# dluvizon/deephar

Measured on NVIDIA H100. Metric: frames/sec (256x256, 16-frame clips, b32), higher is better.
Workload: dtype bf16x3 split (fp32 accumulate, wgmma)

## Files before the change

### deephar_b200/_ffi.py

```python
import ctypes as C
import os

_HERE = os.path.dirname(os.path.abspath(__file__))
LIB_PATH = os.environ.get('DEEPHAR_B200_LIB') or os.path.join(_HERE, 'libdeephar_b200.so')


class DeepharB200Error(RuntimeError):
    pass


class dh_view(C.Structure):
    _fields_ = [('p', C.c_void_p), ('n', C.c_int32), ('h', C.c_int32), ('w', C.c_int32),
                ('c', C.c_int32), ('ld', C.c_int32)]


class dh_conv_desc(C.Structure):
    _fields_ = [('kh', C.c_int32), ('kw', C.c_int32), ('sh', C.c_int32), ('sw', C.c_int32),
                ('pad_same', C.c_int32), ('pre_relu', C.c_int32), ('post_relu', C.c_int32),
                ('n_res', C.c_int32),
                ('pre_scale', C.c_void_p), ('pre_shift', C.c_void_p),
                ('post_scale', C.c_void_p), ('post_shift', C.c_void_p),
                ('res', dh_view * 2),
                ('precision', C.c_int32), ('res_up2x', C.c_int32), ('pool_out', dh_view)]


class dh_frame_src(C.Structure):
    _fields_ = [('data', C.c_uint64), ('h', C.c_int32), ('w', C.c_int32), ('stride', C.c_int32),
                ('x0', C.c_int32), ('y0', C.c_int32), ('cw', C.c_int32), ('ch', C.c_int32), ('hflip', C.c_int32),
                ('kx_off', C.c_int32), ('ky_off', C.c_int32), ('kx_coef_off', C.c_int32), ('ky_coef_off', C.c_int32),
                ('ksx', C.c_int32), ('ksy', C.c_int32)]


class dh_packed_w(C.Structure):
    _fields_ = [('hi', C.c_void_p), ('lo', C.c_void_p), ('cout_pad', C.c_int32), ('k', C.c_int32)]


class dh_conv_plan_info(C.Structure):
    _fields_ = [('path', C.c_int32), ('fallback', C.c_int32), ('workspace_bytes', C.c_int64),
                ('n_mtiles', C.c_int32), ('grid_x', C.c_int32), ('grid_y', C.c_int32), ('bn_cta', C.c_int32),
                ('n_kblocks', C.c_int32), ('stages', C.c_int32), ('cluster', C.c_int32)]


class dh_clip_window(C.Structure):
    _fields_ = [('src', dh_view), ('dst', dh_view), ('ring', C.c_void_p)]


class dh_jpeg_image(C.Structure):
    _fields_ = [('data', C.c_int64), ('coef', C.c_int64 * 3), ('plane', C.c_int64 * 3), ('out', C.c_int64),
                ('h', C.c_int32), ('w', C.c_int32), ('ncomp', C.c_int32), ('hs', C.c_int32), ('vs', C.c_int32),
                ('mcus_x', C.c_int32), ('mcus_y', C.c_int32), ('bw', C.c_int32 * 3), ('bh', C.c_int32 * 3),
                ('qt', C.c_int32 * 3), ('dc', C.c_int32 * 3), ('ac', C.c_int32 * 3), ('nblocks', C.c_int32),
                ('pad', C.c_int32)]


class dh_jpeg_segment(C.Structure):
# ... 111 lines not shown
```

### deephar_b200/csrc/conv_api.cu

```cuda
#include "tc_common.cuh"

namespace {

struct Choice {
    DhConvPath path;
    bool fallback;
    int64_t workspace_bytes;
    tc::PatchPlan patch;
    tc::SepPlan sep;
    tc::TcPlan tcp;
};

int choose_conv(const dh_ctx* ctx, const ConvParams& p, const dh_packed_w* packed, bool separable, int precision,
                Choice* c) {
    const bool packed_hi = packed && packed->hi;
    c->fallback = false;
    c->workspace_bytes = 0;
    if (separable) {
        DH_CHECK_ARG(!p.pool, "dh_sepconv2d_f32: pool_out is not supported by the separable kernels");
        if (packed_hi && dh_plan_sep_tma(ctx, p, packed, precision, &c->sep)) { c->path = DH_PATH_SEP_TMA; return 0; }
    } else {
        if (!p.up1 && !p.pool && dh_conv_smallk_ok(p)) { c->path = DH_PATH_SIMT; return 0; }
        if (ctx->pw_smallk && !p.up1 && dh_pw_smallk_supported(p)) { c->path = DH_PATH_PW_SMALLK; return 0; }
        DH_CHECK_ARG(!p.pool, "dh_conv2d_f32: pool_out is written by the wide pointwise kernel only (1x1, stride 1, "
// ... 47 lines not shown
    q.kh = q.kw = 1; q.sh = q.sw = 1; q.pt = q.pl = 0;
    q.pre_scale = q.pre_shift = nullptr; q.pre_relu = 0;
    q.K = p.Cin;
    dh_launch_conv_simt(q, s);
    DH_LAUNCH_EPILOGUE(ctx, 2);
}

template <class Params>
void tc_info(const dh_ctx* ctx, const tc::Plan<Params>& pl, const tc::TcParams& P, dh_conv_plan_info* info) {
    info->n_mtiles = P.n_mtiles;
    info->grid_x = tc::persistent_gx(ctx, pl.gy, P.n_mtiles);
    info->grid_y = pl.gy;
    info->bn_cta = P.bn_cta;
    info->n_kblocks = P.n_kblocks;
    info->cluster = pl.cluster;
}

int plan_info(const dh_ctx* ctx, const Choice& c, dh_conv_plan_info* info) {
    DH_CHECK_ARG(info, "dh_conv_plan_info: NULL info");
    *info = dh_conv_plan_info{};
    info->path = c.path;
    info->fallback = c.fallback;
    info->workspace_bytes = c.workspace_bytes;
    if (c.path == DH_PATH_TC) {
        tc_info(ctx, c.tcp, c.tcp.k, info);
        info->stages = c.tcp.k.stages;
    }
    if (c.path == DH_PATH_SEP_TMA) tc_info(ctx, c.sep, c.sep.k.t, info);
    if (c.path == DH_PATH_PATCH) tc_info(ctx, c.patch, c.patch.k.t, info);
    return 0;
}

}

extern "C" int dh_conv2d_f32(dh_ctx* ctx, const dh_view* x, const float* w_hwio,
                             const dh_packed_w* packed, const dh_conv_desc* d, const dh_view* out,
                             void* stream) {
    ConvParams p;
    Choice c;
    int rc = plan_conv(ctx, x, nullptr, w_hwio, packed, d, out, false, &p, &c);
    return rc ? rc : launch_choice(ctx, p, c, false, (cudaStream_t)stream);
}

// ... 26 lines not shown
```

### deephar_b200/csrc/conv_sep.cu

```cuda
#include "tc_common.cuh"

namespace tcs {
using namespace tc;
using R = tc::Roles<2, 1>;
constexpr int WARP_EPI0 = R::WARP_EPI0, WARP_TMA = R::WARP_TMA, WARP_PATCH = R::WARP_PATCH, NTHREADS = R::NTHREADS,
              REGS_PROD = R::REGS_PROD, REGS_EPI = R::REGS_EPI, REGS_CTRL = R::REGS_CTRL;

constexpr int NWG = 128;
constexpr int NPW = 1;
constexpr int NA = 4;
constexpr int NB = 3;
constexpr int NP = 3;

template <int KS, int TW, bool SHARE, bool BNPRO, bool LO>
__global__ void __launch_bounds__(NTHREADS, 1)
sep_tma_kernel(const __grid_constant__ SepParams SP, const __grid_constant__ CUtensorMap map_hi,
               const __grid_constant__ CUtensorMap map_lo, const __grid_constant__ CUtensorMap map_x) {
    constexpr int PAD = KS / 2;
    constexpr int PC = TW + 2 * PAD;
    constexpr int NR = 4 + KS - 1;
#ifdef DH_ABLATE
    const int DBG = SP.dbg;
#else
    constexpr int DBG = 0;
#endif
    const TcParams& P = SP.t;
    extern __shared__ __align__(1024) uint8_t smem_raw[];
    if (smem_u32(smem_raw) & 1023u) __trap();
    uint8_t* smem = smem_raw;
    const int tid = threadIdx.x;
    const int warp = tid >> 5, lane = tid & 31;
    constexpr bool want_lo = LO;
    const int b_bytes = P.bn_cta * 64;
    uint8_t* b_ring = smem + NA * 2 * A_BYTES;
    uint8_t* patch0 = b_ring + NB * 2 * b_bytes;
// ... 30 lines not shown
    if (SHARE) cluster_sync_all(); else __syncthreads();

    const int tiles_mine = ((int)P.n_mtiles - (int)blockIdx.x + (int)gridDim.x - 1) / (int)gridDim.x;
    const int total_g = tiles_mine * nkb;
    const int n_own = SHARE ? (total_g - (int)my_rank + 1) / 2 : total_g;

    if (warp < WARP_EPI0) {
        reg_prod<REGS_PROD, R::LAUNCH_REGS>();
        const ConvParams& c = P.c;
        const int w = warp >> 2;
        const int tw = tid & (NWG - 1);
        const int cp = tw & 15;
        const int blk = tw >> 4;
        constexpr int XB = TW / 4;
        const int strip = blk / XB, xb = blk - strip * XB;
        const int fn = (strip * 4) / SP.ry, ry = (strip * 4) - fn * SP.ry;
        const int prr = SP.ry + 2 * PAD;
        const float* pbase0 = reinterpret_cast<const float*>(patch0) +
                             ((size_t)((fn * prr + ry) * PC + xb * 4)) * SBK + cp * 2;
        const int row0 = strip * 4 * TW + xb * 4;
        const float lowb = c.pre_relu ? 0.f : -3.402823466e38f;
        unsigned colmask = 0;
        if (BNPRO) {
#pragma unroll
            for (int q = 0; q < NR; ++q) {
                const int ix = xb * 4 + q - PAD;
                if (ix >= 0 && ix < TW) colmask |= 1u << q;
            }
        }
        float2 wt[KS][KS];
        auto load_taps = [&](int jn) {
            const int gn = SHARE ? 2 * jn + (int)my_rank : jn;
            const int kbn = gn % nkb;
            const float* wp = c.w_dw + kbn * SBK + cp * 2;
#pragma unroll
            for (int a = 0; a < KS; ++a)
#pragma unroll
                for (int b = 0; b < KS; ++b)
                    wt[a][b] = __ldg(reinterpret_cast<const float2*>(wp + (size_t)(a * KS + b) * c.Cin));
        };
        if (w < n_own) load_taps(w);
        for (int j = w; j < n_own; j += NPW) {
            const int pb_i = j % NP;
            const uint32_t pfull = bar_pfull0 + 8 * pb_i, pempty = bar_pempty0 + 8 * pb_i;
            const float* pbase = pbase0 + (size_t)pb_i * (SP.patch_stride / 4);
            const int g = SHARE ? 2 * j + (int)my_rank : j;
            const int ti = g / nkb, kb = g - ti * nkb;
            const int ch = kb * SBK + cp * 2;
            float2 acc[4][4];
#pragma unroll
            for (int o = 0; o < 4; ++o)
#pragma unroll
                for (int q = 0; q < 4; ++q) acc[o][q] = make_float2(0.f, 0.f);
            float2 ps = make_float2(1.f, 1.f), pb = make_float2(0.f, 0.f);
            unsigned rowmask = 0;
            if (BNPRO) {
                ps = __ldg(reinterpret_cast<const float2*>(c.pre_scale + ch));
                pb = __ldg(reinterpret_cast<const float2*>(c.pre_shift + ch));
                const int t = blockIdx.x + ti * gridDim.x;
                const int y0 = SP.fn > 1 ? 0 : ((t * BM) / TW) % c.H;
#pragma unroll
                for (int r = 0; r < NR; ++r) {
                    const int iy = y0 + ry + r - PAD;
                    if (iy >= 0 && iy < c.H) rowmask |= 1u << r;
                }
            }

            if (!(DBG & 2)) mbar_wait_relaxed(pfull, (uint32_t)((j / NP) & 1), (DBG & 2048) ? 32u : 0u);
            auto load_row = [&](int r, float2* in) {
#pragma unroll
                for (int q = 0; q < NR; ++q) {
                    float2 v = *reinterpret_cast<const float2*>(pbase + (r * PC + q) * SBK);
                    if (BNPRO) v = ffma2(v, ps, pb);
                    v = make_float2(fmaxf(v.x, lowb), fmaxf(v.y, lowb));
                    if (BNPRO && !(((rowmask >> r) & 1u) && ((colmask >> q) & 1u))) v = make_float2(0.f, 0.f);
                    in[q] = v;
                }
            };
            if (!(DBG & 1)) {
                float2 inb[2][NR];
                load_row(0, inb[0]);
#pragma unroll
                for (int r = 0; r < NR; ++r) {
                    if (r + 1 < NR) load_row(r + 1, inb[(r + 1) & 1]);
                    const float2* in = inb[r & 1];
#pragma unroll
                    for (int kx = 0; kx < KS; ++kx)
#pragma unroll
                        for (int o = 0; o < 4; ++o) {
                            const int ky = r - o;
                            if (ky >= 0 && ky < KS) {
#pragma unroll
                                for (int q = 0; q < 4; ++q) acc[o][q] = ffma2(wt[ky][kx], in[q + kx], acc[o][q]);
                            }
                        }
                }
            }
            if (j + NPW < n_own) load_taps(j + NPW);
            if (!(DBG & 2)) mbar_arrive(pempty);

            const int s = g % NA;
            const uint32_t it = (uint32_t)(g / NA);
            wait_stage_free(bar_empty0, s, it, (DBG & 2048) ? 32u : 0u);
            uint8_t* a_hi = smem + (size_t)s * (2 * A_BYTES);
            uint8_t* a_lo = a_hi + A_BYTES;
#pragma unroll
            for (int o = 0; o < 4; ++o)
#pragma unroll
                for (int q = 0; q < 4; ++q) {
                    uint32_t hi, lo;
                    split2(acc[o][q].x, acc[o][q].y, hi, lo);
                    const uint32_t off = swz64(row0 + o * TW + q, cp * 2);
                    *reinterpret_cast<uint32_t*>(a_hi + off) = hi;
                    if (want_lo) *reinterpret_cast<uint32_t*>(a_lo + off) = lo;
                }
            fence_proxy_async();
            if (SHARE) {
                asm volatile("bar.sync %0, %1;" ::"r"(1 + w), "r"(NWG) : "memory");
                if (tw == 0) {
                    mbar_arrive(bar_full0 + 8 * s);
                    const uint32_t peer = my_rank ^ 1u;
                    const uint32_t peer_full = mapa_peer(bar_full0 + 8 * s, peer);
                    if (!(DBG & 8)) {
                        bulk_s2peer(mapa_peer(smem_u32(a_hi), peer), smem_u32(a_hi), A_BYTES, peer_full);
                        if (want_lo) bulk_s2peer(mapa_peer(smem_u32(a_lo), peer), smem_u32(a_lo), A_BYTES, peer_full);
                    }
                }
            } else {
                mbar_arrive(bar_full0 + 8 * s);
            }
        }
    } else if (warp < WARP_TMA) {
        reg_inc<REGS_EPI>();
        stage_post<R::NEPI>(P, n0, post, tid - 32 * WARP_EPI0);
        const int wg = (warp - WARP_EPI0) >> 2, wt = tid - 32 * WARP_EPI0 - 128 * wg;
        pp_consumer<SHARE, LO, NA, NB>(P, wg, wt, n0, tiles_mine, make_desc64(smem_u32(smem)), make_desc64(smem_u32(b_ring)),
                                       bar_full0, bar_empty0, bar_fullb0, bar_emptyb0, my_rank, post, DBG);
    } else {
        reg_dec<REGS_CTRL>();
        if (warp == WARP_TMA) {
            if (lane == 0) {
                const uint32_t tx = (DBG & 16) ? 0u : (uint32_t)(want_lo ? 2 : 1) * (uint32_t)b_bytes;
                const uint32_t tx_a = (DBG & 8) ? 0u : (uint32_t)(want_lo ? 2 : 1) * (uint32_t)A_BYTES;
                for (int g = 0; g < total_g; ++g) {
                    const int ti = g / nkb, kb = g - ti * nkb;
                    const int sb = g % NB;
                    const uint32_t itb = (uint32_t)(g / NB);
                    if (itb >= 1) mbar_wait_relaxed(bar_emptyb0 + 8 * sb, (itb - 1) & 1, (DBG & 2048) ? 64u : 0u);
                    const uint32_t full = bar_fullb0 + 8 * sb;
                    mbar_arrive_expect_tx(full, tx);
                    const uint32_t b_hi = smem_u32(b_ring + (size_t)sb * (2 * b_bytes));
// ... 5 lines not shown
                    if (SHARE && (uint32_t)(g & 1) != my_rank) {
                        const int sa = g % NA;
                        wait_stage_free(bar_empty0, sa, (uint32_t)(g / NA));
                        mbar_arrive_expect_tx(bar_full0 + 8 * sa, tx_a);
                    }
                }
            }
        } else if (warp == WARP_PATCH) {
            if (lane == 0 && !(DBG & 2)) {
                const ConvParams& c = P.c;
                auto coords = [&](int j, int& kb, int& nf, int& y0) {
                    const int g = SHARE ? 2 * j + (int)my_rank : j;
                    const int ti = g / nkb;
                    kb = g - ti * nkb;
                    const int t = blockIdx.x + ti * gridDim.x;
                    const int grow = (t * BM) / TW;
                    nf = grow / c.H;
                    y0 = grow - nf * c.H;
                };
                for (int j = 0; j < n_own; ++j) {
                    int kb, nf, y0;
                    coords(j, kb, nf, y0);
                    const int w = j % NP;
                    const int pfd = (DBG & 1024) ? 2 : (DBG & 4096) ? 4 : (DBG & 8192) ? 9 : 0;
                    if (pfd && j + pfd < n_own) {
                        int kb2, nf2, y2;
                        coords(j + pfd, kb2, nf2, y2);
                        tma_prefetch_4d(&map_x, kb2 * SBK, -PAD, y2 - PAD, nf2);
                    }
                    mbar_wait_relaxed(bar_pempty0 + 8 * w, (uint32_t)(((j / NP) & 1) ^ 1), (DBG & 2048) ? 64u : 0u);
                    const uint32_t pf = bar_pfull0 + 8 * w;
// ... 4 lines not shown
        }
    }
    if (SHARE) cluster_sync_all(); else __syncthreads();
}

}

bool dh_plan_sep_tma(const dh_ctx* ctx, const ConvParams& p, const dh_packed_w* packed, int precision, tc::SepPlan* pl) {
    using namespace tc;
    using namespace tcs;
    if (!ctx->sep_tma || !packed->lo || !sep_layer_ok(p, packed)) return false;
    if (!(p.W == 32 || p.W == 16 || p.W == 8)) return false;
    const int tr = BM / p.W;
    if (tr <= p.H ? (p.H % tr) != 0 : (tr % p.H) != 0) return false;
    if ((p.Cin % SBK) != 0 || (p.ldx & 3)) return false;
    SepParams& SP = pl->k;
    TcParams& P = SP.t;
    P.c = p;
    P.c.K = p.Cin;
    P.k_pad = packed->k;
    P.n_kblocks = p.Cin / SBK;
    int gy;
    tile_n(p.Cout, &P.bn_cta, &gy);
    P.precision = (precision == 1) ? 1 : 3;
    P.ks = p.kh;
    P.n_mtiles = (p.M + BM - 1) / BM;
    P.stages = 2;
    const int pad = p.kh / 2;
    SP.ry = tr <= p.H ? tr : p.H;
    SP.fn = tr <= p.H ? 1 : tr / p.H;
    SP.patch_bytes = SBK * 4 * (p.W + 2 * pad) * (SP.ry + 2 * pad) * SP.fn;
    SP.patch_stride = (SP.patch_bytes + 1023) / 1024 * 1024;
#ifdef DH_ABLATE
    SP.dbg = ctx->dbg;
    P.dbg = ctx->dbg;
#else
    SP.dbg = 0;
    P.dbg = 0;
#endif
    pl->smem = (size_t)NA * 2 * A_BYTES + (size_t)NB * 2 * P.bn_cta * 64 + NP * (size_t)SP.patch_stride + 512 +
               POST_SMEM;
    if (pl->smem > SMEM_LIMIT) return false;
    pl->w = packed;
    pl->gy = gy;
    pl->cluster = gy % 2 == 0 && ctx->share_a;
    return true;
}

int dh_launch_sep_tma(const dh_ctx* ctx, const tc::SepPlan& pl, cudaStream_t s) {
    using namespace tc;
    using namespace tcs;
    const TcParams& P = pl.k.t;
    const ConvParams& c = P.c;
    const dh_packed_w* w = pl.w;
    const int pad = P.ks / 2;
    CUtensorMap map_hi, map_lo, map_x;
    if (!make_map_w(&map_hi, w->hi, w->k, w->cout_pad, SBK, P.bn_cta) ||
        !make_map_w(&map_lo, w->lo, w->k, w->cout_pad, SBK, P.bn_cta) ||
        !make_map_x(&map_x, c.x, c.ldx, c.Cin, c.W, c.H, c.N, c.W + 2 * pad, pl.k.ry + 2 * pad, pl.k.fn)) {
        dh_set_error("dh_launch_sep_tma: cuTensorMapEncodeTiled failed");
        return -1;
    }
    return pick<5, 3>(P.ks, [&](auto ks) {
        return pick<32, 16, 8>(c.W, [&](auto tw) {
            return pick<true, false>(pl.cluster, [&](auto share) {
                return pick<true, false>(c.pre_scale != nullptr, [&](auto bnpro) {
                    return pick<true, false>(P.precision == 3, [&](auto lo) {
                        return launch_persistent<sep_tma_kernel<ks(), tw(), share(), bnpro(), lo()>>(
                            "dh_launch_sep_tma", ctx, pl, P.n_mtiles, NTHREADS, s, map_hi, map_lo, map_x);
                    });
                });
            });
        });
    });
}
```

### deephar_b200/csrc/tc_common.cuh

```cuda
#pragma once
#include <cuda.h>
#include <cuda_bf16.h>
#include <type_traits>
#include "common.cuh"
#include "conv_params.cuh"

namespace tc {


constexpr int BM = 128;
constexpr int BK = 64;
constexpr int NPROD = 256;
constexpr int MAX_BN_CTA = 96;
constexpr int ACC_N = MAX_BN_CTA / 2;
constexpr int MH = BM / 64;
template <int Q, int NPW = 2>
struct Roles {
    static constexpr int EPQ = Q;
    static constexpr int NEPI = 128 * Q;
    static constexpr int WARP_EPI0 = 4 * NPW;
    static constexpr int WARP_TMA = WARP_EPI0 + 4 * Q, WARP_PATCH = WARP_TMA + 2;
    static constexpr int NTHREADS = 32 * (WARP_TMA + 4);
    static constexpr int REGS_PROD = Q == 1 ? 168 : (NPW == 1 ? 192 : 88);
    static constexpr int REGS_EPI = Q == 2 && NPW == 2 ? 136 : 144, REGS_CTRL = 32;
    static constexpr int LAUNCH_REGS = NTHREADS <= 512 ? 128 : 96;
    static_assert(128 * NPW * REGS_PROD + NEPI * REGS_EPI + 128 * REGS_CTRL <= NTHREADS * LAUNCH_REGS,
                  "setmaxnreg budget exceeds the CTA's register allocation: the last setmaxnreg.inc would never return");
};
constexpr int A_TILE_BYTES = BM * 128;
constexpr int MAX_STAGES = 4;
// ... 3 lines not shown
    int n_kblocks;
    int bn_cta;
    int stages;
    int precision;
    int ks;
    int k_pad;
    int n_mtiles;
    int dbg;
};

struct SepParams {
    TcParams t;
    int patch_stride;
    int patch_bytes;
    int ry, fn;
    int dbg;
};

struct PatchParams {
    TcParams t;
    int np, patch_stride, patch_bytes;
    int ntaps, ncb;
    int tw;
    int ry, fn;
    int pc, pr;
    int rows_per_frame;
    int kw;
    int pt, pl, sh, sw;
    int vh, vw;
    int mask;
// ... 73 lines not shown
template <> __device__ __forceinline__ void wgmma_bf16<80>(float* d, uint64_t a, uint64_t b, uint32_t acc) {
    asm volatile(
        "{\n .reg .pred p;\n setp.ne.b32 p, %42, 0;\n"
        " wgmma.mma_async.sync.aligned.m64n80k16.f32.bf16.bf16 {%0, %1, %2, %3, %4, %5, %6, %7, %8, %9, %10, %11, %12, %13, %14, %15, %16, %17, %18, %19, %20, %21, %22, %23, %24, %25, %26, %27, %28, %29, %30, %31, %32, %33, %34, %35, %36, %37, %38, %39}, %40, %41, p, 1, 1, 0, 0;\n}"
        : "+f"(d[0]), "+f"(d[1]), "+f"(d[2]), "+f"(d[3]), "+f"(d[4]), "+f"(d[5]), "+f"(d[6]), "+f"(d[7]), "+f"(d[8]), "+f"(d[9]), "+f"(d[10]), "+f"(d[11]), "+f"(d[12]), "+f"(d[13]), "+f"(d[14]), "+f"(d[15]), "+f"(d[16]), "+f"(d[17]), "+f"(d[18]), "+f"(d[19]), "+f"(d[20]), "+f"(d[21]), "+f"(d[22]), "+f"(d[23]), "+f"(d[24]), "+f"(d[25]), "+f"(d[26]), "+f"(d[27]), "+f"(d[28]), "+f"(d[29]), "+f"(d[30]), "+f"(d[31]), "+f"(d[32]), "+f"(d[33]), "+f"(d[34]), "+f"(d[35]), "+f"(d[36]), "+f"(d[37]), "+f"(d[38]), "+f"(d[39])
        : "l"(a), "l"(b), "r"(acc));
}
template <> __device__ __forceinline__ void wgmma_bf16<96>(float* d, uint64_t a, uint64_t b, uint32_t acc) {
    asm volatile(
        "{\n .reg .pred p;\n setp.ne.b32 p, %50, 0;\n"
        " wgmma.mma_async.sync.aligned.m64n96k16.f32.bf16.bf16 {%0, %1, %2, %3, %4, %5, %6, %7, %8, %9, %10, %11, %12, %13, %14, %15, %16, %17, %18, %19, %20, %21, %22, %23, %24, %25, %26, %27, %28, %29, %30, %31, %32, %33, %34, %35, %36, %37, %38, %39, %40, %41, %42, %43, %44, %45, %46, %47}, %48, %49, p, 1, 1, 0, 0;\n}"
        : "+f"(d[0]), "+f"(d[1]), "+f"(d[2]), "+f"(d[3]), "+f"(d[4]), "+f"(d[5]), "+f"(d[6]), "+f"(d[7]), "+f"(d[8]), "+f"(d[9]), "+f"(d[10]), "+f"(d[11]), "+f"(d[12]), "+f"(d[13]), "+f"(d[14]), "+f"(d[15]), "+f"(d[16]), "+f"(d[17]), "+f"(d[18]), "+f"(d[19]), "+f"(d[20]), "+f"(d[21]), "+f"(d[22]), "+f"(d[23]), "+f"(d[24]), "+f"(d[25]), "+f"(d[26]), "+f"(d[27]), "+f"(d[28]), "+f"(d[29]), "+f"(d[30]), "+f"(d[31]), "+f"(d[32]), "+f"(d[33]), "+f"(d[34]), "+f"(d[35]), "+f"(d[36]), "+f"(d[37]), "+f"(d[38]), "+f"(d[39]), "+f"(d[40]), "+f"(d[41]), "+f"(d[42]), "+f"(d[43]), "+f"(d[44]), "+f"(d[45]), "+f"(d[46]), "+f"(d[47])
        : "l"(a), "l"(b), "r"(acc));
}

__device__ __forceinline__ uint64_t make_desc(uint32_t smem_addr) {
    return (uint64_t)((smem_addr >> 4) & 0x3FFF) | (1ull << 16) | ((uint64_t)(1024 >> 4) << 32) | (1ull << 62);
}


__device__ __forceinline__ void split2(float a, float b, uint32_t& hi, uint32_t& lo) {
    __nv_bfloat162 h = __floats2bfloat162_rn(a, b);
    float ra = a - __low2float(h), rb = b - __high2float(h);
    __nv_bfloat162 l = __floats2bfloat162_rn(ra, rb);
    hi = *reinterpret_cast<uint32_t*>(&h);
    lo = *reinterpret_cast<uint32_t*>(&l);
}

__device__ __forceinline__ uint32_t swz(int row, int k) {
    return (uint32_t)(row * 128 + ((((k >> 3) ^ (row & 7)) << 4) | ((k & 7) << 1)));
// ... 21 lines not shown
__device__ __forceinline__ uint32_t swz64(int row, int k) {
    return (uint32_t)(row * 64 + ((((k >> 3) ^ ((row >> 1) & 3)) << 4) | ((k & 7) << 1)));
}

__device__ __forceinline__ float4 lds128(uint32_t a) {
    float4 v;
    asm volatile("ld.shared.v4.f32 {%0, %1, %2, %3}, [%4];" : "=f"(v.x), "=f"(v.y), "=f"(v.z), "=f"(v.w) : "r"(a) : "memory");
    return v;
}

__device__ __forceinline__ void wait_stage_free(uint32_t bar_empty0, int s, uint32_t it, uint32_t ns = 0) {
    if (it >= 1) mbar_wait_relaxed(bar_empty0 + 16 * s + 8 * ((it - 1) & 1), ((it - 1) >> 1) & 1, ns);
}


template <int N>
__device__ __forceinline__ void acc_fence_all(float (&acc)[MH][ACC_N]) {
#pragma unroll
    for (int h = 0; h < MH; ++h)
#pragma unroll
        for (int i = 0; i < N / 2; ++i) acc_fence(acc[h][i]);
}

template <int N, int NK16, bool LO>
__device__ __forceinline__ void wg_issue_kblock(float (&acc)[MH][ACC_N], uint64_t da, uint32_t a_half16, uint32_t alo16,
                                                uint64_t db, uint32_t blo16, bool first) {
    wgmma_fence();
#pragma unroll
    for (int k = 0; k < NK16; ++k) {
        const uint32_t acc0 = (first && k == 0) ? 0u : 1u;
#pragma unroll
        for (int h = 0; h < MH; ++h) {
            const uint64_t a = da + (uint64_t)(h * a_half16 + 2 * k);
            wgmma_bf16<N>(acc[h], a, db + 2 * k, acc0);
            if (LO) {
                wgmma_bf16<N>(acc[h], a + alo16, db + 2 * k, 1u);
                wgmma_bf16<N>(acc[h], a, db + blo16 + 2 * k, 1u);
            }
        }
    }
    wgmma_commit();
}

template <int N, int NK16, bool LO, class Stage, class Release>
__device__ __forceinline__ void wg_tile_n(float (&acc)[MH][ACC_N], int nkb, uint32_t a_half16, uint32_t alo16,
                                          uint32_t blo16, bool mma, Stage& stage, Release& release) {
    for (int kb = 0; kb < nkb; ++kb) {
        uint64_t da, db;
        stage(kb, da, db);
        if (mma) {
            acc_fence_all<N>(acc);
            wg_issue_kblock<N, NK16, LO>(acc, da, a_half16, alo16, db, blo16, kb == 0);
        }
        wgmma_wait<1>();
        acc_fence_all<N>(acc);
        if (kb > 0) release(kb - 1);
    }
    wgmma_wait<0>();
    acc_fence_all<N>(acc);
    release(nkb - 1);
}

template <int NK16, bool LO, class Stage, class Release>
__device__ __forceinline__ void wg_tile(int bn, float (&acc)[MH][ACC_N], int nkb, uint32_t a_half16, uint32_t alo16,
                                        uint32_t blo16, bool mma, Stage&& stage, Release&& release) {
    switch (bn) {
    case 16: wg_tile_n<16, NK16, LO>(acc, nkb, a_half16, alo16, blo16, mma, stage, release); break;
    case 32: wg_tile_n<32, NK16, LO>(acc, nkb, a_half16, alo16, blo16, mma, stage, release); break;
    case 48: wg_tile_n<48, NK16, LO>(acc, nkb, a_half16, alo16, blo16, mma, stage, release); break;
    case 64: wg_tile_n<64, NK16, LO>(acc, nkb, a_half16, alo16, blo16, mma, stage, release); break;
    case 80: wg_tile_n<80, NK16, LO>(acc, nkb, a_half16, alo16, blo16, mma, stage, release); break;
    default: wg_tile_n<96, NK16, LO>(acc, nkb, a_half16, alo16, blo16, mma, stage, release); break;
    }
}

__device__ __forceinline__ void pp_pass(int wg) { asm volatile("bar.arrive %0, 256;" ::"r"(6 + wg) : "memory"); }
__device__ __forceinline__ void pp_wait(int wg) { asm volatile("bar.sync %0, 256;" ::"r"(7 - wg) : "memory"); }

__device__ __forceinline__ void wg_release(uint32_t bar, int wg, int wt, bool remote, uint32_t peer) {
    asm volatile("bar.sync %0, 128;" ::"r"(4 + wg) : "memory");
    if (wt == 0) {
        mbar_arrive(bar);
        if (remote) mbar_arrive_cluster(mapa_peer(bar, peer));
    }
}

__device__ __forceinline__ size_t res1_src(const ConvParams& c, int m) {
    if (!c.up1) return (size_t)m;
    const int hw = c.Ho * c.Wo;
    const int n = m / hw, rem = m - n * hw;
    const int y = rem / c.Wo, x = rem - y * c.Wo;
    return ((size_t)n * (c.Ho >> 1) + (y >> 1)) * (size_t)(c.Wo >> 1) + (size_t)(x >> 1);
}

__device__ __forceinline__ float2 ldg2(const float* p) { return __ldg(reinterpret_cast<const float2*>(p)); }

constexpr int POST_SMEM = 2 * MAX_BN_CTA * 4;
template <int NEPI>
__device__ __forceinline__ void stage_post(const TcParams& P, int n0, float* post, int ct) {
    const ConvParams& c = P.c;
    if (c.post_scale) {
        for (int j = ct; j < P.bn_cta; j += NEPI) {
            const int co = n0 + j;
            post[j] = co < c.Cout ? __ldg(c.post_scale + co) : 0.f;
            post[MAX_BN_CTA + j] = co < c.Cout ? __ldg(c.post_shift + co) : 0.f;
        }
    }
    asm volatile("bar.sync 2, %0;" ::"n"(NEPI) : "memory");
}

__device__ __forceinline__ void prefetch_l2(const float* p) { asm volatile("prefetch.global.L2 [%0];" ::"l"(p)); }
__device__ __forceinline__ void wg_prefetch_res(const TcParams& P, int m0, int n0, int wt) {
    const ConvParams& c = P.c;
#ifdef DH_ABLATE
    if (P.dbg & 32) return;
#endif
    const int m = m0 + wt;
    if (m >= c.M) return;
    const int last = min(P.bn_cta, c.Cout - n0) - 1;
    if (c.res0) {
        const float* r = c.res0 + (size_t)m * c.ldr0 + n0;
        for (int k = 0; k < last; k += 32) prefetch_l2(r + k);
        prefetch_l2(r + last);
    }
    if (c.res1) {
        const float* r = c.res1 + res1_src(c, m) * c.ldr1 + n0;
        for (int k = 0; k < last; k += 32) prefetch_l2(r + k);
        prefetch_l2(r + last);
    }
}

__device__ __forceinline__ void wg_epilogue(const TcParams& P, const float (&acc)[MH][ACC_N], int m0, int n0, int wt,
                                            const float* post) {
    const ConvParams& c = P.c;
#ifdef DH_ABLATE
    if (P.dbg & 32) return;
#endif
    const int rq = 16 * (wt >> 5) + ((wt & 31) >> 2);
    const int c0 = n0 + 2 * (wt & 3);
    const bool v2 = !((c.ldo | c.Cout) & 1) && !(reinterpret_cast<uintptr_t>(c.out) & 7) &&
                    (!c.res0 || (!(c.ldr0 & 1) && !(reinterpret_cast<uintptr_t>(c.res0) & 7))) &&
                    (!c.res1 || (!(c.ldr1 & 1) && !(reinterpret_cast<uintptr_t>(c.res1) & 7)));
    const bool relu = c.post_relu != 0, has_post = c.post_scale != nullptr;
    const int ncol = min(P.bn_cta - 2 * (wt & 3), c.Cout - c0);
    const float* sc = post + (c0 - n0);
    const float* sh = sc + MAX_BN_CTA;
    constexpr int JC = 3;
    static_assert((ACC_N / 4) % JC == 0, "column groups per batch");
#pragma unroll
    for (int h = 0; h < MH; ++h)
#pragma unroll
        for (int hr = 0; hr < 2; ++hr) {
            const int m = m0 + 64 * h + rq + 8 * hr;
            if (m >= c.M) continue;
            float* orow = c.out + (size_t)m * c.ldo + c0;
            const float* r0row = c.res0 ? c.res0 + (size_t)m * c.ldr0 + c0 : nullptr;
            const float* r1row = c.res1 ? c.res1 + res1_src(c, m) * c.ldr1 + c0 : nullptr;
            if (v2) {
#pragma unroll
                for (int j0 = 0; j0 < ACC_N / 4; j0 += JC) {
                    if (8 * j0 >= P.bn_cta) break;
                    float2 ra[JC], rb[JC];
#pragma unroll
                    for (int jj = 0; jj < JC; ++jj) {
                        if (8 * (j0 + jj) < ncol) {
                            if (r0row) ra[jj] = ldg2(r0row + 8 * (j0 + jj));
                            if (r1row) rb[jj] = ldg2(r1row + 8 * (j0 + jj));
                        }
                    }
#pragma unroll
                    for (int jj = 0; jj < JC; ++jj) {
                        const int j = j0 + jj;
                        if (8 * j < ncol) {
                            float2 v = make_float2(acc[h][4 * j + 2 * hr], acc[h][4 * j + 2 * hr + 1]);
                            if (has_post)
                                v = ffma2(v, *reinterpret_cast<const float2*>(sc + 8 * j),
                                          *reinterpret_cast<const float2*>(sh + 8 * j));
                            if (relu) v = make_float2(fmaxf(v.x, 0.f), fmaxf(v.y, 0.f));
                            if (r0row) v = fadd2(v, ra[jj]);
                            if (r1row) v = fadd2(v, rb[jj]);
                            *reinterpret_cast<float2*>(orow + 8 * j) = v;
                        }
                    }
                }
                continue;
            }
#pragma unroll
            for (int j = 0; j < ACC_N / 4; ++j) {
                if (8 * j >= P.bn_cta) break;
#pragma unroll
                for (int e = 0; e < 2; ++e) {
                    const int k = 8 * j + e;
                    if (k < ncol) {
                        float t = acc[h][4 * j + 2 * hr + e];
                        if (has_post) t = fmaf(t, sc[k], sh[k]);
                        if (relu) t = fmaxf(t, 0.f);
                        if (r0row) t += __ldg(r0row + k);
                        if (r1row) t += __ldg(r1row + k);
                        orow[k] = t;
                    }
                }
            }
        }
}

template <bool SHARE, bool LO, int NA, int NB>
__device__ __forceinline__ void pp_consumer(const TcParams& P, int wg, int wt, int n0, int tiles_mine, uint64_t dbase,
                                            uint64_t dbase_b, uint32_t bar_full0, uint32_t bar_empty0,
                                            uint32_t bar_fullb0, uint32_t bar_emptyb0, uint32_t rank, const float* post,
                                            int dbg) {
    static_assert(NA % 2 == 0 || !SHARE, "each A stage has one producing CTA of the pair");
    const int nkb = P.n_kblocks;
    const int b_bytes = P.bn_cta * 64;
    float acc[MH][ACC_N];
    const uint32_t sta16 = (2 * A_BYTES) >> 4, stb16 = (uint32_t)(2 * b_bytes) >> 4, alo16 = A_BYTES >> 4,
                   blo16 = (uint32_t)b_bytes >> 4, half16 = (64 * 64) >> 4;
    for (int ti = wg; ti < tiles_mine; ti += 2) {
        const int g0 = ti * nkb, m0 = ((int)blockIdx.x + ti * (int)gridDim.x) * BM;
        if (ti > 0) pp_wait(wg);
        wg_prefetch_res(P, m0, n0, wt);
        wg_tile<SBK / 16, LO>(
            P.bn_cta, acc, nkb, half16, alo16, blo16, !(dbg & 64),
            [&](int kb, uint64_t& da, uint64_t& db) {
                const int g = g0 + kb, s = g % NA, sb = g % NB;
                if (!(dbg & 128)) mbar_wait(bar_full0 + 8 * s, (uint32_t)(g / NA) & 1);
                mbar_wait(bar_fullb0 + 8 * sb, (uint32_t)(g / NB) & 1);
                if (kb == nkb - 1 && ti + 1 < tiles_mine) pp_pass(wg);
                da = dbase + (uint64_t)((uint32_t)s * sta16);
                db = dbase_b + (uint64_t)((uint32_t)sb * stb16);
            },
            [&](int kb) {
                const int g = g0 + kb, s = g % NA;
                const uint32_t producer = (uint32_t)(s & 1);
                wg_release(bar_empty0 + 16 * s + 8 * ((g / NA) & 1), wg, wt, SHARE && producer != rank, producer);
                if (wt == 0) mbar_arrive(bar_emptyb0 + 8 * (g % NB));
// ... 31 lines not shown
}

static inline bool make_map_x(CUtensorMap* map, const float* x, int ldx, int c, int w, int h, int n, int pc, int pr,
                              int fn) {
    EncodeTiledFn enc = get_encode();
    if (!enc) return false;
    cuuint64_t dims[4] = {(cuuint64_t)c, (cuuint64_t)w, (cuuint64_t)h, (cuuint64_t)n};
    cuuint64_t strides[3] = {(cuuint64_t)ldx * 4, (cuuint64_t)w * ldx * 4, (cuuint64_t)h * w * ldx * 4};
    cuuint32_t box[4] = {(cuuint32_t)SBK, (cuuint32_t)pc, (cuuint32_t)pr, (cuuint32_t)fn};
    cuuint32_t estr[4] = {1, 1, 1, 1};
    return enc(map, CU_TENSOR_MAP_DATA_TYPE_FLOAT32, 4, const_cast<float*>(x), dims, strides, box, estr,
               CU_TENSOR_MAP_INTERLEAVE_NONE, CU_TENSOR_MAP_SWIZZLE_NONE, CU_TENSOR_MAP_L2_PROMOTION_L2_256B,
               CU_TENSOR_MAP_FLOAT_OOB_FILL_NONE) == CUDA_SUCCESS;
}

static inline void tile_n(int cout, int* bn_cta, int* gy) {
    const int cp = (cout + 15) / 16 * 16;
    const int g = (cp + MAX_BN_CTA - 1) / MAX_BN_CTA;
    *bn_cta = ((cp + g - 1) / g + 15) / 16 * 16;
    *gy = g;
}

constexpr size_t SMEM_LIMIT = 227 * 1024;

static inline bool packed_fits(const dh_packed_w* w, int K, int cout) {
    return w->k == dh_tc_k_pad(K) && w->cout_pad == dh_tc_cout_pad(cout);
}

static inline bool bn_pro_aligned(const ConvParams& p) {
    return !p.pre_scale || !((reinterpret_cast<uintptr_t>(p.pre_scale) | reinterpret_cast<uintptr_t>(p.pre_shift)) & 15);
}

static inline bool tc_layer_ok(const ConvParams& p, const dh_packed_w* w, int K) {
// ... 75 lines not shown
```

### include/deephar_b200.h

```cpp
#ifndef DEEPHAR_B200_H
#define DEEPHAR_B200_H

#include <stdint.h>

#ifdef __cplusplus
extern "C" {
#endif

typedef struct dh_view {
    float*  p;
    int32_t n, h, w, c;
    int32_t ld;
} dh_view;

typedef struct dh_conv_desc {
    int32_t kh, kw, sh, sw;
    int32_t pad_same;
    int32_t pre_relu;
    int32_t post_relu;
    int32_t n_res;
    const float* pre_scale;
    const float* pre_shift;
    const float* post_scale;
    const float* post_shift;
// ... 29 lines not shown

int dh_sepconv2d_f32(dh_ctx* ctx, const dh_view* x, const float* w_dw, const float* w_pw,
                     const dh_packed_w* packed_pw, const dh_conv_desc* d, const dh_view* out,
                     void* stream);

typedef struct dh_conv_plan_info {
    int32_t path;
    int32_t fallback;
    int64_t workspace_bytes;
    int32_t n_mtiles;
    int32_t grid_x, grid_y;
    int32_t bn_cta;
    int32_t n_kblocks;
    int32_t stages;
    int32_t cluster;
} dh_conv_plan_info;
int dh_conv2d_plan(dh_ctx* ctx, const dh_view* x, const float* w_hwio, const dh_packed_w* packed,
                   const dh_conv_desc* d, const dh_view* out, dh_conv_plan_info* info);
int dh_sepconv2d_plan(dh_ctx* ctx, const dh_view* x, const float* w_dw, const float* w_pw,
                      const dh_packed_w* packed_pw, const dh_conv_desc* d, const dh_view* out,
                      dh_conv_plan_info* info);

int dh_maxpool2d_f32(dh_ctx* ctx, const dh_view* x, int kh, int kw, int sh, int sw, int pad_same,
                     const dh_view* out, void* stream);
int dh_upsample2x_add_f32(dh_ctx* ctx, const dh_view* a, const dh_view* b, const dh_view* out,
                          void* stream);
int dh_add_n_f32(dh_ctx* ctx, const dh_view* in, int n_in, const float* scale, const float* shift,
                 int relu, const dh_view* out, void* stream);

int dh_softargmax2d_f32(dh_ctx* ctx, const dh_view* h, const dh_view* d, float alpha,
// ... 102 lines not shown
```

Measured before the change: 3723.

## Add 64-row M tile with 144-wide N tile for separable TMA conv

```diff
diff --git a/deephar_b200/_ffi.py b/deephar_b200/_ffi.py
--- a/deephar_b200/_ffi.py
+++ b/deephar_b200/_ffi.py
@@ -38,7 +38,7 @@
 class dh_conv_plan_info(C.Structure):
     _fields_ = [('path', C.c_int32), ('fallback', C.c_int32), ('workspace_bytes', C.c_int64),
                 ('n_mtiles', C.c_int32), ('grid_x', C.c_int32), ('grid_y', C.c_int32), ('bn_cta', C.c_int32),
-                ('n_kblocks', C.c_int32), ('stages', C.c_int32), ('cluster', C.c_int32)]
+                ('n_kblocks', C.c_int32), ('stages', C.c_int32), ('cluster', C.c_int32), ('bm', C.c_int32)]
 
 
 class dh_clip_window(C.Structure):
diff --git a/deephar_b200/csrc/conv_api.cu b/deephar_b200/csrc/conv_api.cu
--- a/deephar_b200/csrc/conv_api.cu
+++ b/deephar_b200/csrc/conv_api.cu
@@ -85,6 +85,7 @@
     info->bn_cta = P.bn_cta;
     info->n_kblocks = P.n_kblocks;
     info->cluster = pl.cluster;
+    info->bm = tc::BM;
 }
 
 int plan_info(const dh_ctx* ctx, const Choice& c, dh_conv_plan_info* info) {
@@ -97,7 +98,10 @@
         tc_info(ctx, c.tcp, c.tcp.k, info);
         info->stages = c.tcp.k.stages;
     }
-    if (c.path == DH_PATH_SEP_TMA) tc_info(ctx, c.sep, c.sep.k.t, info);
+    if (c.path == DH_PATH_SEP_TMA) {
+        tc_info(ctx, c.sep, c.sep.k.t, info);
+        info->bm = c.sep.k.bm;
+    }
     if (c.path == DH_PATH_PATCH) tc_info(ctx, c.patch, c.patch.k.t, info);
     return 0;
 }
diff --git a/deephar_b200/csrc/conv_sep.cu b/deephar_b200/csrc/conv_sep.cu
--- a/deephar_b200/csrc/conv_sep.cu
+++ b/deephar_b200/csrc/conv_sep.cu
@@ -11,14 +11,20 @@
 constexpr int NA = 4;
 constexpr int NB = 3;
 constexpr int NP = 3;
-
-template <int KS, int TW, bool SHARE, bool BNPRO, bool LO>
+#ifdef DH_ABLATE
+constexpr int DBG_TILE64 = 1 << 14, DBG_TILE128 = 1 << 15;
+#endif
+
+template <int TBM, int KS, int TW, bool SHARE, bool BNPRO, bool LO>
 __global__ void __launch_bounds__(NTHREADS, 1)
 sep_tma_kernel(const __grid_constant__ SepParams SP, const __grid_constant__ CUtensorMap map_hi,
                const __grid_constant__ CUtensorMap map_lo, const __grid_constant__ CUtensorMap map_x) {
     constexpr int PAD = KS / 2;
     constexpr int PC = TW + 2 * PAD;
-    constexpr int NR = 4 + KS - 1;
+    constexpr int OR = TBM / 32;
+    constexpr int NR = OR + KS - 1;
+    constexpr int NC = 4 + KS - 1;
+    constexpr int A_BYTES = TBM * 64;
 #ifdef DH_ABLATE
     const int DBG = SP.dbg;
 #else
@@ -79,16 +85,16 @@
         const int blk = tw >> 4;
         constexpr int XB = TW / 4;
         const int strip = blk / XB, xb = blk - strip * XB;
-        const int fn = (strip * 4) / SP.ry, ry = (strip * 4) - fn * SP.ry;
+        const int fn = (strip * OR) / SP.ry, ry = (strip * OR) - fn * SP.ry;
         const int prr = SP.ry + 2 * PAD;
         const float* pbase0 = reinterpret_cast<const float*>(patch0) +
                              ((size_t)((fn * prr + ry) * PC + xb * 4)) * SBK + cp * 2;
-        const int row0 = strip * 4 * TW + xb * 4;
+        const int row0 = strip * OR * TW + xb * 4;
         const float lowb = c.pre_relu ? 0.f : -3.402823466e38f;
         unsigned colmask = 0;
         if (BNPRO) {
 #pragma unroll
-            for (int q = 0; q < NR; ++q) {
+            for (int q = 0; q < NC; ++q) {
                 const int ix = xb * 4 + q - PAD;
                 if (ix >= 0 && ix < TW) colmask |= 1u << q;
             }
@@ -112,9 +118,9 @@
             const int g = SHARE ? 2 * j + (int)my_rank : j;
             const int ti = g / nkb, kb = g - ti * nkb;
             const int ch = kb * SBK + cp * 2;
-            float2 acc[4][4];
-#pragma unroll
-            for (int o = 0; o < 4; ++o)
+            float2 acc[OR][4];
+#pragma unroll
+            for (int o = 0; o < OR; ++o)
 #pragma unroll
                 for (int q = 0; q < 4; ++q) acc[o][q] = make_float2(0.f, 0.f);
             float2 ps = make_float2(1.f, 1.f), pb = make_float2(0.f, 0.f);
@@ -123,7 +129,7 @@
                 ps = __ldg(reinterpret_cast<const float2*>(c.pre_scale + ch));
                 pb = __ldg(reinterpret_cast<const float2*>(c.pre_shift + ch));
                 const int t = blockIdx.x + ti * gridDim.x;
-                const int y0 = SP.fn > 1 ? 0 : ((t * BM) / TW) % c.H;
+                const int y0 = SP.fn > 1 ? 0 : ((t * TBM) / TW) % c.H;
 #pragma unroll
                 for (int r = 0; r < NR; ++r) {
                     const int iy = y0 + ry + r - PAD;
@@ -134,7 +140,7 @@
             if (!(DBG & 2)) mbar_wait_relaxed(pfull, (uint32_t)((j / NP) & 1), (DBG & 2048) ? 32u : 0u);
             auto load_row = [&](int r, float2* in) {
 #pragma unroll
-                for (int q = 0; q < NR; ++q) {
+                for (int q = 0; q < NC; ++q) {
                     float2 v = *reinterpret_cast<const float2*>(pbase + (r * PC + q) * SBK);
                     if (BNPRO) v = ffma2(v, ps, pb);
                     v = make_float2(fmaxf(v.x, lowb), fmaxf(v.y, lowb));
@@ -143,7 +149,7 @@
                 }
             };
             if (!(DBG & 1)) {
-                float2 inb[2][NR];
+                float2 inb[2][NC];
                 load_row(0, inb[0]);
 #pragma unroll
                 for (int r = 0; r < NR; ++r) {
@@ -152,7 +158,7 @@
 #pragma unroll
                     for (int kx = 0; kx < KS; ++kx)
 #pragma unroll
-                        for (int o = 0; o < 4; ++o) {
+                        for (int o = 0; o < OR; ++o) {
                             const int ky = r - o;
                             if (ky >= 0 && ky < KS) {
 #pragma unroll
@@ -170,7 +176,7 @@
             uint8_t* a_hi = smem + (size_t)s * (2 * A_BYTES);
             uint8_t* a_lo = a_hi + A_BYTES;
 #pragma unroll
-            for (int o = 0; o < 4; ++o)
+            for (int o = 0; o < OR; ++o)
 #pragma unroll
                 for (int q = 0; q < 4; ++q) {
                     uint32_t hi, lo;
@@ -197,9 +203,9 @@
         }
     } else if (warp < WARP_TMA) {
         reg_inc<REGS_EPI>();
-        stage_post<R::NEPI>(P, n0, post, tid - 32 * WARP_EPI0);
+        stage_post<R::NEPI, bn_max(TBM)>(P, n0, post, tid - 32 * WARP_EPI0);
         const int wg = (warp - WARP_EPI0) >> 2, wt = tid - 32 * WARP_EPI0 - 128 * wg;
-        pp_consumer<SHARE, LO, NA, NB>(P, wg, wt, n0, tiles_mine, make_desc64(smem_u32(smem)), make_desc64(smem_u32(b_ring)),
+        pp_consumer<SHARE, LO, NA, NB, TBM>(P, wg, wt, n0, tiles_mine, make_desc64(smem_u32(smem)), make_desc64(smem_u32(b_ring)),
                                        bar_full0, bar_empty0, bar_fullb0, bar_emptyb0, my_rank, post, DBG);
     } else {
         reg_dec<REGS_CTRL>();
@@ -235,7 +241,7 @@
                     const int ti = g / nkb;
                     kb = g - ti * nkb;
                     const int t = blockIdx.x + ti * gridDim.x;
-                    const int grow = (t * BM) / TW;
+                    const int grow = (t * TBM) / TW;
                     nf = grow / c.H;
                     y0 = grow - nf * c.H;
                 };
@@ -270,23 +276,24 @@
     const int tr = BM / p.W;
     if (tr <= p.H ? (p.H % tr) != 0 : (tr % p.H) != 0) return false;
     if ((p.Cin % SBK) != 0 || (p.ldx & 3)) return false;
+    int bn64, gy64;
+    tile_n(p.Cout, &bn64, &gy64, MAX_BN_CTA64);
+    const bool fits64 = ctx->share_a && bn64 == MAX_BN_CTA64 && gy64 % 2 == 0;
+    bool t64 = fits64 && p.Cin >= 288;
+#ifdef DH_ABLATE
+    if (ctx->dbg & DBG_TILE64) t64 = fits64;
+    if (ctx->dbg & DBG_TILE128) t64 = false;
+#endif
     SepParams& SP = pl->k;
     TcParams& P = SP.t;
     P.c = p;
     P.c.K = p.Cin;
     P.k_pad = packed->k;
     P.n_kblocks = p.Cin / SBK;
-    int gy;
-    tile_n(p.Cout, &P.bn_cta, &gy);
     P.precision = (precision == 1) ? 1 : 3;
     P.ks = p.kh;
-    P.n_mtiles = (p.M + BM - 1) / BM;
     P.stages = 2;
     const int pad = p.kh / 2;
-    SP.ry = tr <= p.H ? tr : p.H;
-    SP.fn = tr <= p.H ? 1 : tr / p.H;
-    SP.patch_bytes = SBK * 4 * (p.W + 2 * pad) * (SP.ry + 2 * pad) * SP.fn;
-    SP.patch_stride = (SP.patch_bytes + 1023) / 1024 * 1024;
 #ifdef DH_ABLATE
     SP.dbg = ctx->dbg;
     P.dbg = ctx->dbg;
@@ -294,12 +301,24 @@
     SP.dbg = 0;
     P.dbg = 0;
 #endif
-    pl->smem = (size_t)NA * 2 * A_BYTES + (size_t)NB * 2 * P.bn_cta * 64 + NP * (size_t)SP.patch_stride + 512 +
-               POST_SMEM;
-    if (pl->smem > SMEM_LIMIT) return false;
+    auto geometry = [&](int bm) {
+        int gy;
+        tile_n(p.Cout, &P.bn_cta, &gy, bn_max(bm));
+        const int trb = bm / p.W;
+        SP.bm = bm;
+        P.n_mtiles = (p.M + bm - 1) / bm;
+        SP.ry = trb <= p.H ? trb : p.H;
+        SP.fn = trb <= p.H ? 1 : trb / p.H;
+        SP.patch_bytes = SBK * 4 * (p.W + 2 * pad) * (SP.ry + 2 * pad) * SP.fn;
+        SP.patch_stride = (SP.patch_bytes + 1023) / 1024 * 1024;
+        pl->smem = (size_t)NA * 2 * (bm * 64) + (size_t)NB * 2 * P.bn_cta * 64 + NP * (size_t)SP.patch_stride + 512 +
+                   post_smem(bm);
+        pl->gy = gy;
+        return pl->smem <= SMEM_LIMIT;
+    };
+    if (!(t64 && geometry(BM64)) && !geometry(BM)) return false;
     pl->w = packed;
-    pl->gy = gy;
-    pl->cluster = gy % 2 == 0 && ctx->share_a;
+    pl->cluster = pl->gy % 2 == 0 && ctx->share_a;
     return true;
 }
 
@@ -319,10 +338,13 @@
     }
     return pick<5, 3>(P.ks, [&](auto ks) {
         return pick<32, 16, 8>(c.W, [&](auto tw) {
-            return pick<true, false>(pl.cluster, [&](auto share) {
-                return pick<true, false>(c.pre_scale != nullptr, [&](auto bnpro) {
-                    return pick<true, false>(P.precision == 3, [&](auto lo) {
-                        return launch_persistent<sep_tma_kernel<ks(), tw(), share(), bnpro(), lo()>>(
+            return pick<true, false>(c.pre_scale != nullptr, [&](auto bnpro) {
+                return pick<true, false>(P.precision == 3, [&](auto lo) {
+                    if (pl.k.bm == BM64)
+                        return launch_persistent<sep_tma_kernel<BM64, ks(), tw(), true, bnpro(), lo()>>(
+                            "dh_launch_sep_tma", ctx, pl, P.n_mtiles, NTHREADS, s, map_hi, map_lo, map_x);
+                    return pick<true, false>(pl.cluster, [&](auto share) {
+                        return launch_persistent<sep_tma_kernel<BM, ks(), tw(), share(), bnpro(), lo()>>(
                             "dh_launch_sep_tma", ctx, pl, P.n_mtiles, NTHREADS, s, map_hi, map_lo, map_x);
                     });
                 });
diff --git a/deephar_b200/csrc/tc_common.cuh b/deephar_b200/csrc/tc_common.cuh
--- a/deephar_b200/csrc/tc_common.cuh
+++ b/deephar_b200/csrc/tc_common.cuh
@@ -14,6 +14,9 @@
 constexpr int MAX_BN_CTA = 96;
 constexpr int ACC_N = MAX_BN_CTA / 2;
 constexpr int MH = BM / 64;
+constexpr int BM64 = 64;
+constexpr int MAX_BN_CTA64 = 144;
+constexpr int bn_max(int bm) { return bm == BM64 ? MAX_BN_CTA64 : MAX_BN_CTA; }
 template <int Q, int NPW = 2>
 struct Roles {
     static constexpr int EPQ = Q;
@@ -47,6 +50,7 @@
     int patch_stride;
     int patch_bytes;
     int ry, fn;
+    int bm;
     int dbg;
 };
 
@@ -150,6 +154,14 @@
         : "l"(a), "l"(b), "r"(acc));
 }
 
+template <> __device__ __forceinline__ void wgmma_bf16<144>(float* d, uint64_t a, uint64_t b, uint32_t acc) {
+    asm volatile(
+        "{\n .reg .pred p;\n setp.ne.b32 p, %74, 0;\n"
+        " wgmma.mma_async.sync.aligned.m64n144k16.f32.bf16.bf16 {%0, %1, %2, %3, %4, %5, %6, %7, %8, %9, %10, %11, %12, %13, %14, %15, %16, %17, %18, %19, %20, %21, %22, %23, %24, %25, %26, %27, %28, %29, %30, %31, %32, %33, %34, %35, %36, %37, %38, %39, %40, %41, %42, %43, %44, %45, %46, %47, %48, %49, %50, %51, %52, %53, %54, %55, %56, %57, %58, %59, %60, %61, %62, %63, %64, %65, %66, %67, %68, %69, %70, %71}, %72, %73, p, 1, 1, 0, 0;\n}"
+        : "+f"(d[0]), "+f"(d[1]), "+f"(d[2]), "+f"(d[3]), "+f"(d[4]), "+f"(d[5]), "+f"(d[6]), "+f"(d[7]), "+f"(d[8]), "+f"(d[9]), "+f"(d[10]), "+f"(d[11]), "+f"(d[12]), "+f"(d[13]), "+f"(d[14]), "+f"(d[15]), "+f"(d[16]), "+f"(d[17]), "+f"(d[18]), "+f"(d[19]), "+f"(d[20]), "+f"(d[21]), "+f"(d[22]), "+f"(d[23]), "+f"(d[24]), "+f"(d[25]), "+f"(d[26]), "+f"(d[27]), "+f"(d[28]), "+f"(d[29]), "+f"(d[30]), "+f"(d[31]), "+f"(d[32]), "+f"(d[33]), "+f"(d[34]), "+f"(d[35]), "+f"(d[36]), "+f"(d[37]), "+f"(d[38]), "+f"(d[39]), "+f"(d[40]), "+f"(d[41]), "+f"(d[42]), "+f"(d[43]), "+f"(d[44]), "+f"(d[45]), "+f"(d[46]), "+f"(d[47]), "+f"(d[48]), "+f"(d[49]), "+f"(d[50]), "+f"(d[51]), "+f"(d[52]), "+f"(d[53]), "+f"(d[54]), "+f"(d[55]), "+f"(d[56]), "+f"(d[57]), "+f"(d[58]), "+f"(d[59]), "+f"(d[60]), "+f"(d[61]), "+f"(d[62]), "+f"(d[63]), "+f"(d[64]), "+f"(d[65]), "+f"(d[66]), "+f"(d[67]), "+f"(d[68]), "+f"(d[69]), "+f"(d[70]), "+f"(d[71])
+        : "l"(a), "l"(b), "r"(acc));
+}
+
 __device__ __forceinline__ uint64_t make_desc(uint32_t smem_addr) {
     return (uint64_t)((smem_addr >> 4) & 0x3FFF) | (1ull << 16) | ((uint64_t)(1024 >> 4) << 32) | (1ull << 62);
 }
@@ -201,23 +213,23 @@
 }
 
 
-template <int N>
-__device__ __forceinline__ void acc_fence_all(float (&acc)[MH][ACC_N]) {
-#pragma unroll
-    for (int h = 0; h < MH; ++h)
+template <int N, int MHT, int ACCN>
+__device__ __forceinline__ void acc_fence_all(float (&acc)[MHT][ACCN]) {
+#pragma unroll
+    for (int h = 0; h < MHT; ++h)
 #pragma unroll
         for (int i = 0; i < N / 2; ++i) acc_fence(acc[h][i]);
 }
 
-template <int N, int NK16, bool LO>
-__device__ __forceinline__ void wg_issue_kblock(float (&acc)[MH][ACC_N], uint64_t da, uint32_t a_half16, uint32_t alo16,
+template <int N, int NK16, bool LO, int MHT, int ACCN>
+__device__ __forceinline__ void wg_issue_kblock(float (&acc)[MHT][ACCN], uint64_t da, uint32_t a_half16, uint32_t alo16,
                                                 uint64_t db, uint32_t blo16, bool first) {
     wgmma_fence();
 #pragma unroll
     for (int k = 0; k < NK16; ++k) {
         const uint32_t acc0 = (first && k == 0) ? 0u : 1u;
 #pragma unroll
-        for (int h = 0; h < MH; ++h) {
+        for (int h = 0; h < MHT; ++h) {
             const uint64_t a = da + (uint64_t)(h * a_half16 + 2 * k);
             wgmma_bf16<N>(acc[h], a, db + 2 * k, acc0);
             if (LO) {
@@ -229,8 +241,8 @@
     wgmma_commit();
 }
 
-template <int N, int NK16, bool LO, class Stage, class Release>
-__device__ __forceinline__ void wg_tile_n(float (&acc)[MH][ACC_N], int nkb, uint32_t a_half16, uint32_t alo16,
+template <int N, int NK16, bool LO, int MHT, int ACCN, class Stage, class Release>
+__device__ __forceinline__ void wg_tile_n(float (&acc)[MHT][ACCN], int nkb, uint32_t a_half16, uint32_t alo16,
                                           uint32_t blo16, bool mma, Stage& stage, Release& release) {
     for (int kb = 0; kb < nkb; ++kb) {
         uint64_t da, db;
@@ -248,16 +260,20 @@
     release(nkb - 1);
 }
 
-template <int NK16, bool LO, class Stage, class Release>
-__device__ __forceinline__ void wg_tile(int bn, float (&acc)[MH][ACC_N], int nkb, uint32_t a_half16, uint32_t alo16,
+template <int NK16, bool LO, int MHT, int ACCN, class Stage, class Release>
+__device__ __forceinline__ void wg_tile(int bn, float (&acc)[MHT][ACCN], int nkb, uint32_t a_half16, uint32_t alo16,
                                         uint32_t blo16, bool mma, Stage&& stage, Release&& release) {
-    switch (bn) {
-    case 16: wg_tile_n<16, NK16, LO>(acc, nkb, a_half16, alo16, blo16, mma, stage, release); break;
-    case 32: wg_tile_n<32, NK16, LO>(acc, nkb, a_half16, alo16, blo16, mma, stage, release); break;
-    case 48: wg_tile_n<48, NK16, LO>(acc, nkb, a_half16, alo16, blo16, mma, stage, release); break;
-    case 64: wg_tile_n<64, NK16, LO>(acc, nkb, a_half16, alo16, blo16, mma, stage, release); break;
-    case 80: wg_tile_n<80, NK16, LO>(acc, nkb, a_half16, alo16, blo16, mma, stage, release); break;
-    default: wg_tile_n<96, NK16, LO>(acc, nkb, a_half16, alo16, blo16, mma, stage, release); break;
+    if constexpr (ACCN == MAX_BN_CTA64 / 2) {
+        wg_tile_n<MAX_BN_CTA64, NK16, LO>(acc, nkb, a_half16, alo16, blo16, mma, stage, release);
+    } else {
+        switch (bn) {
+        case 16: wg_tile_n<16, NK16, LO>(acc, nkb, a_half16, alo16, blo16, mma, stage, release); break;
+        case 32: wg_tile_n<32, NK16, LO>(acc, nkb, a_half16, alo16, blo16, mma, stage, release); break;
+        case 48: wg_tile_n<48, NK16, LO>(acc, nkb, a_half16, alo16, blo16, mma, stage, release); break;
+        case 64: wg_tile_n<64, NK16, LO>(acc, nkb, a_half16, alo16, blo16, mma, stage, release); break;
+        case 80: wg_tile_n<80, NK16, LO>(acc, nkb, a_half16, alo16, blo16, mma, stage, release); break;
+        default: wg_tile_n<96, NK16, LO>(acc, nkb, a_half16, alo16, blo16, mma, stage, release); break;
+        }
     }
 }
 
@@ -282,28 +298,30 @@
 
 __device__ __forceinline__ float2 ldg2(const float* p) { return __ldg(reinterpret_cast<const float2*>(p)); }
 
-constexpr int POST_SMEM = 2 * MAX_BN_CTA * 4;
-template <int NEPI>
+constexpr int post_smem(int bm) { return 2 * bn_max(bm) * 4; }
+constexpr int POST_SMEM = post_smem(BM);
+template <int NEPI, int BNMAX = MAX_BN_CTA>
 __device__ __forceinline__ void stage_post(const TcParams& P, int n0, float* post, int ct) {
     const ConvParams& c = P.c;
     if (c.post_scale) {
         for (int j = ct; j < P.bn_cta; j += NEPI) {
             const int co = n0 + j;
             post[j] = co < c.Cout ? __ldg(c.post_scale + co) : 0.f;
-            post[MAX_BN_CTA + j] = co < c.Cout ? __ldg(c.post_shift + co) : 0.f;
+            post[BNMAX + j] = co < c.Cout ? __ldg(c.post_shift + co) : 0.f;
         }
     }
     asm volatile("bar.sync 2, %0;" ::"n"(NEPI) : "memory");
 }
 
 __device__ __forceinline__ void prefetch_l2(const float* p) { asm volatile("prefetch.global.L2 [%0];" ::"l"(p)); }
+template <int TBM = BM>
 __device__ __forceinline__ void wg_prefetch_res(const TcParams& P, int m0, int n0, int wt) {
     const ConvParams& c = P.c;
 #ifdef DH_ABLATE
     if (P.dbg & 32) return;
 #endif
     const int m = m0 + wt;
-    if (m >= c.M) return;
+    if (wt >= TBM || m >= c.M) return;
     const int last = min(P.bn_cta, c.Cout - n0) - 1;
     if (c.res0) {
         const float* r = c.res0 + (size_t)m * c.ldr0 + n0;
@@ -317,7 +335,8 @@
     }
 }
 
-__device__ __forceinline__ void wg_epilogue(const TcParams& P, const float (&acc)[MH][ACC_N], int m0, int n0, int wt,
+template <int MHT, int ACCN>
+__device__ __forceinline__ void wg_epilogue(const TcParams& P, const float (&acc)[MHT][ACCN], int m0, int n0, int wt,
                                             const float* post) {
     const ConvParams& c = P.c;
 #ifdef DH_ABLATE
@@ -331,11 +350,11 @@
     const bool relu = c.post_relu != 0, has_post = c.post_scale != nullptr;
     const int ncol = min(P.bn_cta - 2 * (wt & 3), c.Cout - c0);
     const float* sc = post + (c0 - n0);
-    const float* sh = sc + MAX_BN_CTA;
+    const float* sh = sc + 2 * ACCN;
     constexpr int JC = 3;
-    static_assert((ACC_N / 4) % JC == 0, "column groups per batch");
-#pragma unroll
-    for (int h = 0; h < MH; ++h)
+    static_assert((ACCN / 4) % JC == 0, "column groups per batch");
+#pragma unroll
+    for (int h = 0; h < MHT; ++h)
 #pragma unroll
         for (int hr = 0; hr < 2; ++hr) {
             const int m = m0 + 64 * h + rq + 8 * hr;
@@ -345,7 +364,7 @@
             const float* r1row = c.res1 ? c.res1 + res1_src(c, m) * c.ldr1 + c0 : nullptr;
             if (v2) {
 #pragma unroll
-                for (int j0 = 0; j0 < ACC_N / 4; j0 += JC) {
+                for (int j0 = 0; j0 < ACCN / 4; j0 += JC) {
                     if (8 * j0 >= P.bn_cta) break;
                     float2 ra[JC], rb[JC];
 #pragma unroll
@@ -373,7 +392,7 @@
                 continue;
             }
 #pragma unroll
-            for (int j = 0; j < ACC_N / 4; ++j) {
+            for (int j = 0; j < ACCN / 4; ++j) {
                 if (8 * j >= P.bn_cta) break;
 #pragma unroll
                 for (int e = 0; e < 2; ++e) {
@@ -391,7 +410,7 @@
         }
 }
 
-template <bool SHARE, bool LO, int NA, int NB>
+template <bool SHARE, bool LO, int NA, int NB, int TBM = BM>
 __device__ __forceinline__ void pp_consumer(const TcParams& P, int wg, int wt, int n0, int tiles_mine, uint64_t dbase,
                                             uint64_t dbase_b, uint32_t bar_full0, uint32_t bar_empty0,
                                             uint32_t bar_fullb0, uint32_t bar_emptyb0, uint32_t rank, const float* post,
@@ -399,13 +418,14 @@
     static_assert(NA % 2 == 0 || !SHARE, "each A stage has one producing CTA of the pair");
     const int nkb = P.n_kblocks;
     const int b_bytes = P.bn_cta * 64;
-    float acc[MH][ACC_N];
-    const uint32_t sta16 = (2 * A_BYTES) >> 4, stb16 = (uint32_t)(2 * b_bytes) >> 4, alo16 = A_BYTES >> 4,
+    constexpr int a_bytes = TBM * 64;
+    float acc[TBM / 64][bn_max(TBM) / 2];
+    const uint32_t sta16 = (2 * a_bytes) >> 4, stb16 = (uint32_t)(2 * b_bytes) >> 4, alo16 = a_bytes >> 4,
                    blo16 = (uint32_t)b_bytes >> 4, half16 = (64 * 64) >> 4;
     for (int ti = wg; ti < tiles_mine; ti += 2) {
-        const int g0 = ti * nkb, m0 = ((int)blockIdx.x + ti * (int)gridDim.x) * BM;
+        const int g0 = ti * nkb, m0 = ((int)blockIdx.x + ti * (int)gridDim.x) * TBM;
         if (ti > 0) pp_wait(wg);
-        wg_prefetch_res(P, m0, n0, wt);
+        wg_prefetch_res<TBM>(P, m0, n0, wt);
         wg_tile<SBK / 16, LO>(
             P.bn_cta, acc, nkb, half16, alo16, blo16, !(dbg & 64),
             [&](int kb, uint64_t& da, uint64_t& db) {
@@ -467,9 +487,9 @@
                CU_TENSOR_MAP_FLOAT_OOB_FILL_NONE) == CUDA_SUCCESS;
 }
 
-static inline void tile_n(int cout, int* bn_cta, int* gy) {
+static inline void tile_n(int cout, int* bn_cta, int* gy, int max_bn = MAX_BN_CTA) {
     const int cp = (cout + 15) / 16 * 16;
-    const int g = (cp + MAX_BN_CTA - 1) / MAX_BN_CTA;
+    const int g = (cp + max_bn - 1) / max_bn;
     *bn_cta = ((cp + g - 1) / g + 15) / 16 * 16;
     *gy = g;
 }
diff --git a/include/deephar_b200.h b/include/deephar_b200.h
--- a/include/deephar_b200.h
+++ b/include/deephar_b200.h
@@ -67,6 +67,7 @@
     int32_t n_kblocks;
     int32_t stages;
     int32_t cluster;
+    int32_t bm;
 } dh_conv_plan_info;
 int dh_conv2d_plan(dh_ctx* ctx, const dh_view* x, const float* w_hwio, const dh_packed_w* packed,
                    const dh_conv_desc* d, const dh_view* out, dh_conv_plan_info* info);
```

New measurement: 3859 (median of 6 runs). +3.7%, better.
